# KhaoulaAguech/pl-fem-vectoriel

Hardware: AMD Instinct MI355X
Metric: eigenmodes/sec (assembly+solve), 7-core P2 mesh, 10 modes; |Δn_eff| vs ref (higher is better)
Workload: dtype f64

## Files before the change

### pl_fem_vectoriel_amd/csrc/device.h

```cpp
#pragma once
#include <hip/hip_runtime.h>

#include <cstdint>
#include <functional>
#include <string>
#include <type_traits>
#include <vector>

#include "../../include/plfem.h"
#include "internal.h"
#include "plan.h"

namespace plfem {

constexpr size_t PIN_POST = 0;
constexpr size_t PIN_RESID = 2048;
constexpr size_t PIN_CORE_QP = 4000;
constexpr size_t PIN_COUNTERS = 4096;
constexpr int PIN_COUNTERS_N = 2 * 4;
constexpr size_t PIN_CORES = 6144;
constexpr size_t PIN_PROJ = 8192;
static_assert(PIN_POST + 5 * PLFEM_MAX_NCV <= PIN_RESID, "pinned layout: post-processing sums");
static_assert(PIN_RESID + 3 * PLFEM_MAX_NCV <= PIN_CORE_QP, "pinned layout: residual check");
static_assert(PIN_CORE_QP + 1 <= PIN_COUNTERS, "pinned layout: core-point counter");
// ... 21 lines not shown
  } while (0)

struct plfem_ctx {
  const plfem::Symbolic* S = nullptr;
  const plfem::LaunchPlan* plan = nullptr;
  int device = 0;
  hipStream_t stream = nullptr;
  std::string err;
  int nv = 0, ne = 0, N = 0, nnz = 0, nsolve = 0, L = 0, nfronts = 0, max_ncv = 0;
  int dpn = 2, sh = 1;
  int64_t fnodes_total = 0;
  int64_t n2 = 0;
  int32_t* d_forder = nullptr;
  plfem::FrontRec* d_frec = nullptr;
  int2* d_tiles = nullptr;
  plfem::SweepJob* d_blk = nullptr;
  int32_t *d_tsorted = nullptr, *d_edof = nullptr, *d_rowptr = nullptr, *d_colind = nullptr;
  int32_t *d_slot_row = nullptr, *d_nptr = nullptr, *d_nadj = nullptr, *d_interior = nullptr;
  uint8_t* d_nloc = nullptr;
  uint8_t* d_bmask = nullptr;
  double* d_doflocs = nullptr;
  int32_t *d_fs2 = nullptr, *d_fm = nullptr;
  int64_t *d_fnode_ptr = nullptr, *d_foff = nullptr;
  int32_t *d_fnodes = nullptr, *d_cinv0 = nullptr, *d_cinv1 = nullptr;
  int32_t *d_epos = nullptr, *d_leaf_elem_ptr = nullptr, *d_leaf_elems = nullptr;
  double* d_cores = nullptr;
  double* d_elem = nullptr;
  double* d_vals[PLFEM_BLK_COUNT] = {nullptr};
  double* d_front = nullptr;
  double* d_schur = nullptr;
  int64_t arena_doubles = 0;
  int64_t* d_soff = nullptr;
  double* d_fvec = nullptr;
  double *d_u0 = nullptr, *d_u1 = nullptr;
  double* d_xl = nullptr;
  int32_t* d_npos = nullptr;
  int32_t* d_prow = nullptr;
  double *d_wbuf = nullptr, *d_rbuf = nullptr;
  double* d_dinv = nullptr;
  double* d_delta = nullptr;
  double* d_fvec2 = nullptr;
  int32_t* d_counters = nullptr;
  double *d_V = nullptr, *d_BV = nullptr, *d_V2 = nullptr, *d_BV2 = nullptr;
  double *d_w = nullptr, *d_bw = nullptr, *d_t1 = nullptr, *d_t2 = nullptr;
  double *d_hblk = nullptr, *d_G = nullptr, *d_Rinv = nullptr;
  double *d_h = nullptr, *d_hacc = nullptr, *d_partial = nullptr, *d_scal = nullptr, *d_S = nullptr;
  double* d_Hcols = nullptr;
  uint8_t* d_coremask = nullptr;
  double* d_post = nullptr;
  size_t post_doubles = 0;
  size_t partial_doubles = 0;
  double* h_pinned = nullptr;
  size_t h_pinned_bytes = 0;
  double* h_staging = nullptr;
  size_t h_staging_bytes = 0;
  double* h_slots = nullptr;
  char* slab = nullptr;
  size_t slab_off = 0, slab_bytes = 0;
  bool own_slab = false;
  int64_t workspace_need = 0;
  bool assembled = false, factored = false;
  hipEvent_t ev_step[2] = {nullptr, nullptr};
  bool defer_sync = false;
  hipStream_t copy_stream = nullptr;
  hipEvent_t ev_copy = nullptr;
  hipEvent_t ev_upload = nullptr;
  bool upload_pending = false;
  bool prof_on = false;
  unsigned prof_toggle = 0;
  int prof_n = 0, prof_max = 0;
  std::vector<hipEvent_t> prof_ev;
  std::vector<int> prof_slot;
  std::vector<double> prof_rbytes;
  int refine_steps = 0;
  void (*test_post_factor)(plfem_ctx*) = nullptr;
  double test_perturb = 0.0;
  int max_block_p = plfem::BLOCK_P;
  double sigma = 0.0;
  hipEvent_t ev[plfem::PH_COUNT][2] = {};
  bool ev_used[plfem::PH_COUNT] = {};
  double* modes_dev = nullptr;
  int modes_k = 0;
};

namespace {
template <class Owner>
int check_launch(Owner* owner, const char* what) {
  const hipError_t e = hipGetLastError();
  if (e == hipSuccess) return PLFEM_OK;
  owner->err = std::string(what) + ": " + hipGetErrorString(e);
  return PLFEM_EHIP;
}

int wait_for_upload(plfem_ctx* c) {
  if (!c->upload_pending) return PLFEM_OK;
  HIP_TRY(c, hipStreamWaitEvent(c->stream, c->ev_upload, 0));
  c->upload_pending = false;
  return PLFEM_OK;
}

hipError_t phase_begin(plfem_ctx* c, plfem::Phase ph) { return hipEventRecord(c->ev[ph][0], c->stream); }
hipError_t phase_end(plfem_ctx* c, plfem::Phase ph) {
  const hipError_t e = hipEventRecord(c->ev[ph][1], c->stream);
  if (e == hipSuccess) c->ev_used[ph] = true;
  return e;
}
double phase_us(const plfem_ctx* c, plfem::Phase ph) {
  float ms = 0;
  return (c->ev_used[ph] && hipEventElapsedTime(&ms, c->ev[ph][0], c->ev[ph][1]) == hipSuccess) ? ms * 1e3 : 0.0;
}
}

namespace plfem {

inline int prof_open(plfem_ctx* c, int slot, double bytes) {
  if (!c->prof_on || c->prof_n >= c->prof_max) return -1;
  while ((int)c->prof_ev.size() < 2 * (c->prof_n + 1)) {
    hipEvent_t e;
    if (hipEventCreate(&e) != hipSuccess) return -1;
    c->prof_ev.push_back(e);
  }
  const int id = c->prof_n++;
  c->prof_slot.push_back(slot);
  c->prof_rbytes.push_back(bytes);
  (void)hipEventRecord(c->prof_ev[2 * id], c->stream);
  return id;
}
inline void prof_close(plfem_ctx* c, int id) {
  if (id >= 0) (void)hipEventRecord(c->prof_ev[2 * id + 1], c->stream);
}

template <int V, int... Rest, class F>
inline void with_constant(int v, F&& f) {
  if constexpr (sizeof...(Rest) == 0) f(std::integral_constant<int, V>());
  else if (v == V) f(std::integral_constant<int, V>());
  else with_constant<Rest...>(v, f);
}

inline int ceil_div(int64_t a, int64_t b) { return (int)((a + b - 1) / b); }
inline int basis_cols(int max_ncv) { return max_ncv + 1 + BLOCK_P; }
inline int proj_cols(int max_ncv) { return basis_cols(max_ncv) + 8; }

void launch_element_matrices(plfem_ctx* c, int ncore, double eps_core, double eps_clad, double k0, double alpha_p);
void launch_element_matrices_scalar(plfem_ctx* c, int ncore, double eps_core, double eps_clad, double k0);
double launch_delta_eps_mass(plfem_ctx* c, int ncore, double eps_core, double eps_clad);
void launch_csr_gather(plfem_ctx* c);
void launch_pattern_fill(plfem_ctx* c);
void launch_spmv(plfem_ctx* c, int which, int P, const double* x, double* y, int64_t ld);
int launch_spmv_b_block_il(plfem_ctx* c, const double* x_interleaved, double* y, int64_t ld, double* gram = nullptr);
inline int spmv_workgroups(int N) { return ceil_div(N, SPMV_WG_ROWS); }
inline size_t gram_partial_doubles(int N) { return (size_t)BLOCK_P * BLOCK_P * spmv_workgroups(N); }
void launch_residuals(plfem_ctx* c, int k, const double* lam_host, const double* evecs, double* out_host);
void launch_factor(plfem_ctx* c, double sigma, int stop_level = -1, int stop_step = 0, int stop_stage = 0);
void launch_solve(plfem_ctx* c, int P, const double* rhs, double* x, int64_t ldx, bool rhs_in_front_order = false);
inline int sweep_ldv(int m) { return (m + 2) & ~1; }
inline size_t sweep_dynamic_lds(int P, int m) { return sizeof(double) * P * sweep_ldv(m); }
inline size_t sweep_lds(int P, int m) { return sweep_dynamic_lds(P, m) + sizeof(double) * 8 * P * 64; }
void solve_refined(plfem_ctx* c, int P, const double* b, double* y, int64_t ld, bool b_in_front_order, int steps, double* ta,
                   double* tb, double* dy);
void launch_panel_dot(plfem_ctx* c, int P, const double* Pm, int ncols, const double* W, int64_t ldw, double* h, int ldh,
                      double* hacc = nullptr, int ldacc = 0);
inline int panel_chunks(int64_t n2) { return ceil_div(n2, PANEL_CHUNK); }
inline size_t panel_dot_partial_doubles(int64_t n2, int ncols) { return (size_t)panel_chunks(n2) * ncols * BLOCK_P; }
void launch_panel_axpy(plfem_ctx* c, int P, const double* Pm, int ncols, const double* H, int ldh, double* W, int64_t ldw,
                       double* w_interleaved = nullptr);
void launch_dot(plfem_ctx* c, const double* a, const double* b, double* out);
void launch_scale_store(plfem_ctx* c, const double* w, const double* bw, const double* beta2, double* v, double* bv,
                        double* beta_out);
void launch_axpby(plfem_ctx* c, int64_t n, double a, const double* x, double b, const double* y, double* z);
void launch_rotate(plfem_ctx* c, const double* V, int m, const double* Smat, int ldS, int p, double* out);
void launch_first_pass_block(plfem_ctx* c, const double* BVm, const double* Vm, int ncols, double* W, int64_t ldw, double* Hout, int ldh);
inline int first_pass_segments(int64_t n2) { return ceil_div(n2, FIRST_ROWS); }
inline size_t first_pass_partial_doubles(int64_t n2) { return (size_t)FIRST_COLS * BLOCK_P * first_pass_segments(n2); }
void launch_chol_from_partials(plfem_ctx* c, int nchunks, double* Tblk, int ldT, double* Rinv);
void launch_chol_block(plfem_ctx* c, const double* G, int ldg, double* Tblk, int ldT, double* Rinv);
void launch_block_scale(plfem_ctx* c, const double* W, const double* BW, int64_t ldw, const double* Rinv, double* Vn,
                        double* BVn, int64_t ldv, const double* exp_src = nullptr, int exp_n = 0, double* exp_dst = nullptr,
                        int32_t* cnt_dst = nullptr, double* bv_front = nullptr);
void launch_start_field(plfem_ctx* c, int nvec, double* out);
void launch_post(plfem_ctx* c, int k, double* evecs, int ncore, double* out_host, double* frac_core, double* modes_int);
void post_enqueue(plfem_ctx* c, int k, double* evecs, int ncore, double* modes_int, const std::function<void(int, int)>* group_done);
void post_finish(plfem_ctx* c, int k, double* out_host, double* frac_core);
void resid_enqueue(plfem_ctx* c, int k, const double* lam_host, const double* evecs);
void resid_finish(plfem_ctx* c, int k, double* out_host);
inline int post_blocks(int N) { return ceil_div(N, POST_ROWS); }
inline size_t post_sum_doubles(int N, int modes) { return (size_t)POST_SUMS * modes * (post_blocks(N) + 1); }
inline size_t resid_sum_doubles(int N, int modes) { return (size_t)RESID_SUMS * modes * (post_blocks(N) + 1); }

}
```

### pl_fem_vectoriel_amd/csrc/kernels_front.hip

```cpp
#include <algorithm>

#include <type_traits>

#include "device.h"

namespace plfem {
namespace {

typedef double v4d __attribute__((ext_vector_type(4)));

__device__ __forceinline__ double* schur_of(int f, const int64_t* __restrict__ soff, double* __restrict__ schur, int64_t arena) {
  const int level = 31 - __clz(f + 1);
  return schur + (level & 1) * arena + soff[f];
}

template <int sh>
__global__ __launch_bounds__(256) void k_leaf_assemble(
    int first_front, int ne, double sigma, const int32_t* __restrict__ fs2, const int32_t* __restrict__ fm,
    const int64_t* __restrict__ foff, const int64_t* __restrict__ soff,
    const int64_t* __restrict__ fnode_ptr, const int32_t* __restrict__ fnodes,
    const int32_t* __restrict__ leaf_elem_ptr, const int32_t* __restrict__ leaf_elems,
    const int32_t* __restrict__ epos, const double* __restrict__ elem, double* __restrict__ front,
    double* __restrict__ schur, int64_t arena) {
  const int lf = blockIdx.x;
  const int f = first_front + lf;
  const int m = fm[f], s2 = fs2[f], b2 = m - s2;
  constexpr int dpn = sh + 1;
  double* F = front + foff[f];
  double* S = schur_of(f, soff, schur, arena);
  auto at = [&](int i, int j) -> int64_t { return j < s2 ? (int64_t)j * m + i : (i >= s2 ? -2 - ((int64_t)(j - s2) * b2 + (i - s2)) : -1); };
  const int tid = threadIdx.x;
  const int32_t* fn = fnodes + fnode_ptr[f];
  for (int q = tid; q < (m >> sh); q += 256)
    if (fn[q] < 0) {
      for (int cc = 0; cc < dpn; ++cc) {
        const int d = dpn * q + cc;
        if (d < s2) F[(int64_t)d * m + d] = 1.0;
        else S[(int64_t)(d - s2) * b2 + (d - s2)] = 1.0;
      }
    }
  __syncthreads();
  constexpr int nd = 6 * dpn;
  const int adof = tid / nd, bdof = tid % nd;
  const int a = adof >> sh, ca = adof & sh, b = bdof >> sh, cb = bdof & sh;
  const bool worker = tid < nd * nd;
  const int blk_a = (ca == 0 && cb == 0) ? PLFEM_BLK_AXX : (ca == 0) ? PLFEM_BLK_AXY : (cb == 0) ? PLFEM_BLK_AYX : PLFEM_BLK_AYY;
  const bool diag_blk = ca == cb;
  constexpr int EB = 8;
  for (int q0 = leaf_elem_ptr[lf]; q0 < leaf_elem_ptr[lf + 1]; q0 += EB) {
    const int nb = min(EB, leaf_elem_ptr[lf + 1] - q0);
    int64_t dst[EB];
    double val[EB];
#pragma unroll
    for (int t = 0; t < EB; ++t) {
      dst[t] = -1;
      val[t] = 0.0;
      if (worker && t < nb) {
        const int e = leaf_elems[q0 + t];
        const int pa = epos[(size_t)(q0 + t) * 6 + a], pb = epos[(size_t)(q0 + t) * 6 + b];
        const double* em = elem + (size_t)e * ELEM_STRIDE + a * 6 + b;
        double v = em[blk_a * 36];
        if (diag_blk) v -= sigma * em[PLFEM_BLK_MINV * 36];
        if (pa >= 0 && pb >= 0) { dst[t] = at(dpn * pa + ca, dpn * pb + cb); val[t] = v; }
      }
    }
#pragma unroll
    for (int t = 0; t < EB; ++t) {
      if (t < nb) {
        if (dst[t] >= 0) F[dst[t]] += val[t];
        else if (dst[t] <= -2) S[-2 - dst[t]] += val[t];
        __syncthreads();
      }
    }
  }
}

template <int sh>
__global__ __launch_bounds__(256) void k_front_gather(
    const int2* __restrict__ tiles, const int32_t* __restrict__ fs2, const int32_t* __restrict__ fm,
    const int64_t* __restrict__ foff, const int64_t* __restrict__ soff, const int64_t* __restrict__ fnode_ptr,
    const int32_t* __restrict__ fnodes, const int32_t* __restrict__ cinv0, const int32_t* __restrict__ cinv1,
    double* __restrict__ front, double* __restrict__ schur, int64_t arena) {
  const int2 job = tiles[blockIdx.x];
  const int f = job.x;
  const int m = fm[f], s2 = fs2[f], b2 = m - s2;
  constexpr int dpn = sh + 1;
  const int i = (job.y & 0xffff) * 64 + (threadIdx.x & 63);
  const int j0 = ((job.y >> 16) * 4 + (threadIdx.x >> 6)) * 16;
  if (i >= m || j0 >= m) return;
  if (j0 >= s2 && i < s2) return;
  const int64_t np = fnode_ptr[f];
  const int qi = i >> sh, ci = i & sh;
  const int c0i = cinv0[np + qi], c1i = cinv1[np + qi];
  const bool dummy_i = fnodes[np + qi] < 0;
  const int ch0 = 2 * f + 1, ch1 = 2 * f + 2;
  const int b0 = fm[ch0] - fs2[ch0], b1 = fm[ch1] - fs2[ch1];
  const double* S0 = schur_of(ch0, soff, schur, arena);
  const double* S1 = schur_of(ch1, soff, schur, arena);
  double* F = front + foff[f];
  double* S = schur_of(f, soff, schur, arena);
  int c0j[16 >> sh], c1j[16 >> sh];
#pragma unroll
  for (int q = 0; q < (16 >> sh); ++q) {
    c0j[q] = cinv0[np + (j0 >> sh) + q];
    c1j[q] = cinv1[np + (j0 >> sh) + q];
  }
  double v[16];
#pragma unroll
  for (int jj = 0; jj < 16; ++jj) {
    const int cj = jj & sh, q = jj >> sh;
    double a = 0.0, b = 0.0;
    if (c0i >= 0 && c0j[q] >= 0) {
      const int bi = dpn * c0i + ci, bj = dpn * c0j[q] + cj;
      a = S0[(int64_t)min(bi, bj) * b0 + max(bi, bj)];
    }
    if (c1i >= 0 && c1j[q] >= 0) {
      const int bi = dpn * c1i + ci, bj = dpn * c1j[q] + cj;
      b = S1[(int64_t)min(bi, bj) * b1 + max(bi, bj)];
    }
    v[jj] = a + b;
  }
#pragma unroll
  for (int jj = 0; jj < 16; ++jj) {
    const int j = j0 + jj;
    const double val = (dummy_i && i == j) ? 1.0 : v[jj];
    if (j0 < s2) F[(int64_t)j * m + i] = val;
    else S[(int64_t)(j - s2) * b2 + (i - s2)] = val;
  }
}

__device__ __forceinline__ double fast_rcp(double d) {
  double r = __builtin_amdgcn_rcp(d);
  r = fma(fma(-d, r, 1.0), r, r);
  return fma(fma(-d, r, 1.0), r, r);
}

__device__ __forceinline__ double lane_xor16(double v, bool odd_row) {
  const int lo = __double2loint(v), hi = __double2hiint(v);
  const auto a = __builtin_amdgcn_permlane16_swap(lo, lo, false, false);
  const auto b = __builtin_amdgcn_permlane16_swap(hi, hi, false, false);
  return __hiloint2double(odd_row ? b[0] : b[1], odd_row ? a[0] : a[1]);
}

__device__ __forceinline__ void pair_step(double a, double b, double c, double thr, double rep, bool past_first, bool past_second,
                                          double y0, double y1, const double (&ra)[4], const double (&rb)[4],
                                          double (&v)[4], double& d0, double& d1, double& od, int& nper) {
  const double p = b * b;
  const double det = fma(a, c, -p) - fma(b, b, -p);
  const double s = fmax(fmax(fabs(a), fabs(c)), fabs(b));
  if (p * fabs(det) <= (a * a) * (s * s)) {
    if (__builtin_expect(!(fabs(a) >= thr), 0)) {
      a = (a < 0.0) ? -rep : rep;
      nper += 1;
    }
    const double r1 = fast_rcp(a);
    const double g = b * r1;
    double d2 = fma(-g, b, c);
    if (__builtin_expect(!(fabs(d2) >= thr), 0)) {
      d2 = (d2 < 0.0) ? -rep : rep;
      nper += 1;
    }
    const double r2 = fast_rcp(d2);
    const double l0 = past_first ? y0 * r1 : 0.0;
    const double l1 = past_second ? fma(-l0, b, y1) * r2 : 0.0;
#pragma unroll
    for (int cc = 0; cc < 4; ++cc) v[cc] = fma(-l1, fma(-g, ra[cc], rb[cc]), fma(-l0, ra[cc], v[cc]));
    d0 = r1;
    d1 = r2;
    od = 0.0;
    asm volatile("" ::: "memory");
  } else {
    double dt = det;
    if (__builtin_expect(!(fabs(dt) >= thr * s), 0)) {
      dt = (dt < 0.0) ? -rep * s : rep * s;
      nper += 1;
    }
    const double rd = fast_rcp(dt);
    const double x11 = c * rd, x12 = -b * rd, x22 = a * rd;
    const double l0 = past_second ? fma(y0, x11, y1 * x12) : 0.0;
    const double l1 = past_second ? fma(y0, x12, y1 * x22) : 0.0;
#pragma unroll
    for (int cc = 0; cc < 4; ++cc) v[cc] = fma(-l1, rb[cc], fma(-l0, ra[cc], v[cc]));
    d0 = x11;
    d1 = x22;
    od = x12;
    asm volatile("" ::: "memory");
  }
}

struct PivotLds {
  double row[2][2][NB];
  double col[2][2][NB];
  double rmax[NB];
};

__device__ __forceinline__ void ldl_pivot_block(const double* src, int64_t ld, int nbk, int tid,
                                                double (*tile)[NB + 1], double* __restrict__ sDd, double* __restrict__ sDo,
                                                PivotLds& S, int32_t* __restrict__ counters) {
  static_assert(NB == 32, "thread map of ldl_pivot_block");
  const int i = tid & 31, cg = tid >> 5;
  double v[4];
  double rmax = 0.0;
#pragma unroll
  for (int cc = 0; cc < 4; ++cc) {
    const int c = 4 * cg + cc;
    v[cc] = (i < nbk && c < nbk) ? src[(int64_t)c * ld + i] : (i == c ? 1.0 : 0.0);
    rmax = fmax(rmax, fabs(v[cc]));
  }
  __syncthreads();
  tile[cg][i] = rmax;
  __syncthreads();
  if (tid < NB) {
    double r = 0.0;
#pragma unroll
    for (int g = 0; g < 8; ++g) r = fmax(r, fmax(tile[g][tid], tile[g][tid ^ 1]));
    S.rmax[tid] = r;
  }
  double dd = 1.0, od = 0.0;
  int nper = 0;
#pragma unroll
  for (int q = 0; q < NB / 2; ++q) {
    const int k = 2 * q, cgk = k >> 2, pc = k & 3, buf = q & 1;
    if (k >= nbk) break;
    if (cg == cgk) {
      S.col[buf][0][i] = v[pc];
// ... 366 lines not shown
  {
    PanelOperands po;
    po.load(tile, sDd, sDo, nbn, lr, lk);
    po.rows(bq, nbn, t0, m, ibase0 + lr, lk, Wn, Yn, F);
  }
  for (int ibase = ibase0 + n_pan * 64; ibase < m; ibase += n_pan * 64) {
    int ml = m;
    int64_t pl = pbase;
    asm volatile("" : "+s"(ml), "+s"(pl) : : "memory");
    strip(ibase, bq, std::false_type(), ml, pl);
    asm volatile("" ::: "memory");
    PanelOperands po;
    po.load(tile, sDd, sDo, nbn, lr, lk);
    po.rows(bq, nbn, t0, ml, ibase + lr, lk, wbuf_next + pl, rbuf_next + pl, F);
  }
}

template <int MODE>
__global__ __launch_bounds__(256) __attribute__((amdgpu_waves_per_eu(3, 3))) void k_ldl_update(
    int un, int n_inv, int n_look, int n_pan, const int2* __restrict__ tiles, const int32_t* __restrict__ forder,
    const FrontRec* __restrict__ frec, int kb,
    const int32_t* __restrict__ fs2, const int32_t* __restrict__ fm, const int64_t* __restrict__ foff,
    const int64_t* __restrict__ soff, const int64_t* __restrict__ fnode_ptr, double* __restrict__ front,
    double* __restrict__ schur, int64_t arena, const double* __restrict__ dinv, double* __restrict__ dinv_next,
    double* __restrict__ delta, const double* __restrict__ wbuf, const double* __restrict__ rbuf,
    const double* __restrict__ wbuf_prev, const double* __restrict__ rbuf_prev, double* __restrict__ wbuf_next,
    double* __restrict__ rbuf_next, int32_t* __restrict__ counters) {
  int bid = blockIdx.x;
  if (bid < n_look * n_pan) {
    const FrontRec R = frec[bid / n_pan];
    ldl_column_block<MODE>(R, bid % n_pan, n_pan, kb, front, dinv_next, delta, wbuf, rbuf, wbuf_prev, rbuf_prev, wbuf_next,
                           rbuf_next, counters);
    return;
  }
  bid -= n_look * n_pan;
  if (bid < un) {
    ldl_update_tile<MODE>(tiles[bid], kb, fs2, fm, foff, soff, fnode_ptr, front, schur, arena, wbuf, rbuf, wbuf_prev, rbuf_prev);
    return;
  }
  bid -= un;
  const int f = forder[bid / (n_inv + 1)];
  const int sub = bid % (n_inv + 1);
  if (sub < n_inv) {
    __shared__ double part[3 * 8 * 64];
    ldl_invrow_block(f, sub, kb, fs2, fm, foff, front, dinv, part);
    return;
  }
  const int s2 = fs2[f];
  const int k0 = kb * NB;
  if (k0 >= s2) return;
  const int nbk = min(NB, s2 - k0);
  const int m = fm[f];
  double* F = front + foff[f];
  const double* D = dinv + (int64_t)f * NB * NB;
  for (int q = threadIdx.x; q < NB * NB; q += 256) {
    const int i = q & (NB - 1), c = q >> 5;
    if (i < nbk && c < nbk) F[(int64_t)(k0 + c) * m + (k0 + i)] = (i >= c) ? D[i + c * NB] : D[c + i * NB];
  }
}

__device__ __forceinline__ void mirror_x_block(const int2 job, const int32_t* __restrict__ fs2, const int32_t* __restrict__ fm,
                                               const int64_t* __restrict__ foff, double* __restrict__ front,
                                               double (*tile)[33]) {
  const int f = job.x, k0 = job.y * NB;
  const int m = fm[f], s2 = fs2[f];
  const int nbk = min(NB, s2 - k0);
  double* F = front + foff[f];
  const int tx = threadIdx.x & 31, ty = threadIdx.x >> 5;
  for (int c0 = 0; c0 < k0; c0 += 32) {
    for (int yy = ty; yy < 32; yy += 8)
      tile[yy][tx] = (yy < nbk) ? F[(int64_t)(k0 + yy) * m + c0 + tx] : 0.0;
    __syncthreads();
    for (int yy = ty; yy < 32; yy += 8)
      if (tx < nbk) F[(int64_t)(c0 + yy) * m + k0 + tx] = tile[tx][yy];
    __syncthreads();
  }
}

__global__ __launch_bounds__(256) void k_form_z_mirror(const int2* __restrict__ jobs, int nz, const int32_t* __restrict__ fs2,
                                                       const int32_t* __restrict__ fm, const int64_t* __restrict__ foff,
                                                       double* __restrict__ front) {
  __shared__ double lds[4][32][33];
  const int2 job = jobs[blockIdx.x];
  if ((int)blockIdx.x >= nz) {
    mirror_x_block(job, fs2, fm, foff, front, lds[0]);
    return;
  }
  const int f = job.x;
  const int m = fm[f], s2 = fs2[f];
  const int b2 = m - s2;
  const int wave = threadIdx.x >> 6, lane = threadIdx.x & 63;
  const int b0 = (job.y * 2 + (wave & 1)) * 32;
  const bool rows_on = b0 < b2;
  double* F = front + foff[f];
  double* FZ = F + (int64_t)m * s2;
  const int lr = lane & 15, lk = lane >> 4;
  const bool bv1 = b0 + 16 < b2;
  double (*tile)[33] = lds[wave];
  for (int cstep = 0; cstep < s2; cstep += 64) {
    const int c0 = cstep + 32 * (wave >> 1);
    const bool on = rows_on && c0 < s2;
    const bool cv1 = c0 + 16 < s2;
    v4d acc[2][2];
    for (int tb = 0; tb < 2; ++tb)
      for (int tc = 0; tc < 2; ++tc) acc[tb][tc] = (v4d){0.0, 0.0, 0.0, 0.0};
    if (on) {
      const int cA = c0 + lr, cB = c0 + 16 + lr;
      for (int j0 = c0; j0 < s2; j0 += 16) {
        double a0[4], a1[4], x0[4], x1[4];
#pragma unroll
        for (int t = 0; t < 4; ++t) {
          const int j = j0 + 4 * t + lk;
          a0[t] = F[(int64_t)j * m + s2 + b0 + lr];
          a1[t] = bv1 ? F[(int64_t)j * m + s2 + b0 + 16 + lr] : 0.0;
          x0[t] = (j >= cA) ? F[(int64_t)j * m + cA] : 0.0;
          x1[t] = (cv1 && j >= cB) ? F[(int64_t)j * m + cB] : 0.0;
        }
#pragma unroll
        for (int t = 0; t < 4; ++t) {
          acc[0][0] = __builtin_amdgcn_mfma_f64_16x16x4f64(a0[t], x0[t], acc[0][0], 0, 0, 0);
          acc[0][1] = __builtin_amdgcn_mfma_f64_16x16x4f64(a0[t], x1[t], acc[0][1], 0, 0, 0);
          acc[1][0] = __builtin_amdgcn_mfma_f64_16x16x4f64(a1[t], x0[t], acc[1][0], 0, 0, 0);
          acc[1][1] = __builtin_amdgcn_mfma_f64_16x16x4f64(a1[t], x1[t], acc[1][1], 0, 0, 0);
        }
      }
      for (int tb = 0; tb < 2; ++tb)
        for (int tc = 0; tc < 2; ++tc)
#pragma unroll
          for (int r = 0; r < 4; ++r) {
            const int bb = 16 * tb + lk + 4 * r, cc = 16 * tc + lr;
            tile[cc][bb] = acc[tb][tc][r];
            if ((tb == 0 || bv1) && (tc == 0 || cv1)) FZ[(int64_t)(b0 + bb) * s2 + (c0 + cc)] = acc[tb][tc][r];
          }
    }
    __syncthreads();
    if (on) {
      const int bb = lane & 31;
#pragma unroll 4
      for (int cc = lane >> 5; cc < 32; cc += 2)
        if (b0 + bb < b2 && c0 + cc < s2) F[(int64_t)(c0 + cc) * m + s2 + b0 + bb] = tile[cc][bb];
    }
  }
}

}

void launch_factor(plfem_ctx* c, double sigma, int stop_level, int stop_step, int stop_stage) {
  hipStream_t st = c->stream;
  const LaunchPlan& plan = *c->plan;
  (void)hipMemsetAsync(c->d_counters, 0, 4 * sizeof(int32_t), st);
  for (int lev = c->L; lev >= 0; --lev) {
    const LevelInfo& li = plan.levels[lev];
    if (lev == c->L) {
      const int64_t lo = c->S->foff[li.first], hi = c->S->foff[li.first + li.count];
      (void)hipMemsetAsync(c->d_front + lo, 0, sizeof(double) * (size_t)(hi - lo), st);
      int64_t sch = 0;
      for (int f = li.first; f < li.first + li.count; ++f) {
        const int64_t b2 = (int64_t)c->dpn * c->S->fb[f];
        sch = std::max(sch, c->S->soff[f] + b2 * b2);
      }
      (void)hipMemsetAsync(c->d_schur + (size_t)(lev & 1) * c->arena_doubles, 0, sizeof(double) * (size_t)sch, st);
      with_constant<0, 1>(c->sh, [&](auto sh) {
        hipLaunchKernelGGL(k_leaf_assemble<decltype(sh)::value>, dim3(li.count), dim3(256), 0, st, li.first, c->ne, sigma, c->d_fs2,
                           c->d_fm, c->d_foff, c->d_soff, c->d_fnode_ptr, c->d_fnodes, c->d_leaf_elem_ptr, c->d_leaf_elems, c->d_epos,
                           c->d_elem, c->d_front, c->d_schur, c->arena_doubles);
      });
    } else if (li.gather_n > 0) {
      with_constant<0, 1>(c->sh, [&](auto sh) {
        hipLaunchKernelGGL(k_front_gather<decltype(sh)::value>, dim3(li.gather_n), dim3(256), 0, st, c->d_tiles + li.gather_off,
                           c->d_fs2, c->d_fm, c->d_foff, c->d_soff, c->d_fnode_ptr, c->d_fnodes, c->d_cinv0, c->d_cinv1, c->d_front,
                           c->d_schur, c->arena_doubles);
      });
    }
    if (lev == stop_level && stop_stage == 0) return;
    const int steps = (li.max_s2 + NB - 1) / NB;
    const int32_t* ford = c->d_forder + li.first;
    const FrontRec* frec = c->d_frec + li.first;
    const int* hs2 = plan.forder_s2.data() + li.first;
    const int* hpm = plan.forder_maxm.data() + li.first;
    for (int kb = 0; kb < steps; ++kb) {
      const bool stop_here = (lev == stop_level && kb == stop_step);
      const int k0 = kb * NB;
      int nact = 0;
      {
        int lo = 0, hi = li.count;
        while (lo < hi) { int mid = (lo + hi) / 2; if (hs2[mid] > k0) lo = mid + 1; else hi = mid; }
        nact = lo;
      }
      if (nact == 0) break;
      const size_t third = (size_t)2 * plan.level_nodes_max * NB;
      const int64_t base = 2 * c->S->fnode_ptr[li.first] * NB;
      double* wb0 = c->d_wbuf - base;
      double* rb0 = c->d_rbuf - base;
      double* wb = wb0 + (kb % 3) * third;
      double* rb = rb0 + (kb % 3) * third;
      double* wb_prev = wb0 + ((kb + 2) % 3) * third;
      double* rb_prev = rb0 + ((kb + 2) % 3) * third;
      double* wb_next = wb0 + ((kb + 1) % 3) * third;
      double* rb_next = rb0 + ((kb + 1) % 3) * third;
      double* dinv_cur = c->d_dinv + (size_t)(kb & 1) * c->nfronts * NB * NB;
      double* dinv_nxt = c->d_dinv + (size_t)((kb + 1) & 1) * c->nfronts * NB * NB;
      auto panel_wgs = [&](int rows_below, int cap) {
        int n = std::max(1, rows_below > 0 ? (rows_below + 63) / 64 : 0);
        return li.count > 64 ? std::min(n, cap) : n;
      };
      if (kb == 0) {
        const int n_pan0 = panel_wgs(hpm[nact - 1] - 16, 2);
        hipLaunchKernelGGL(k_ldl_first_panel, dim3(nact, n_pan0), dim3(256), 0, st, frec, c->d_front, dinv_cur, c->d_delta, wb, rb,
                           c->d_counters);
      }
      if (stop_here && stop_stage >= 1 && stop_stage <= 2) return;
      const int un = plan.upd_n[li.step0 + kb];
      const int n_inv = kb > 0 ? (k0 + 15) / 16 : 0;
      const int2* ut = c->d_tiles + plan.upd_off[li.step0 + kb];
      int n_look = 0;
      {
        int lo = 0, hi = nact;
        while (lo < hi) { int mid = (lo + hi) / 2; if (hs2[mid] > k0 + NB) lo = mid + 1; else hi = mid; }
        n_look = lo;
      }
      const int cap = li.count >= 1024 ? 1 : 4;
      const int n_pan = n_look > 0 ? panel_wgs(hpm[n_look - 1] - (k0 + NB) - 16, cap) : 1;
      const unsigned gridB = (unsigned)(n_look * n_pan + un + nact * (n_inv + 1));
      with_constant<0, 1>(kb & 1, [&](auto mode) {
        hipLaunchKernelGGL(k_ldl_update<decltype(mode)::value>, dim3(gridB), dim3(256), 0, st, un, n_inv, n_look, n_pan, ut, ford,
                           frec, kb, c->d_fs2, c->d_fm, c->d_foff, c->d_soff, c->d_fnode_ptr, c->d_front, c->d_schur, c->arena_doubles,
                           dinv_cur, dinv_nxt, c->d_delta, wb, rb, mode ? wb_prev : wb, mode ? rb_prev : rb, wb_next, rb_next,
                           c->d_counters);
      });
      if (stop_here && (stop_stage == 3 || stop_stage == 4)) return;
    }
    if (stop_level >= 0 && li.formz_n + li.mirrorx_n > 0)
      hipLaunchKernelGGL(k_form_z_mirror, dim3(li.formz_n + li.mirrorx_n), dim3(256), 0, st, c->d_tiles + li.formz_off, li.formz_n,
                         c->d_fs2, c->d_fm, c->d_foff, c->d_front);
    if (lev == stop_level && stop_stage == 5) return;
  }
  if (stop_level < 0 && plan.formz_all_n + plan.mirrorx_all_n > 0)
    hipLaunchKernelGGL(k_form_z_mirror, dim3(plan.formz_all_n + plan.mirrorx_all_n), dim3(256), 0, st, c->d_tiles + plan.formz_all_off,
                       plan.formz_all_n, c->d_fs2, c->d_fm, c->d_foff, c->d_front);
}

}
```

### pl_fem_vectoriel_amd/csrc/plan.h

```cpp
#pragma once
#include <cstdint>
#include <functional>
#include <memory>
#include <utility>
#include <vector>

namespace plfem {

template <class T>
struct default_init_allocator : std::allocator<T> {
  template <class U>
  struct rebind { using other = default_init_allocator<U>; };
  using std::allocator<T>::allocator;
  template <class U>
  void construct(U* ptr) noexcept { ::new (static_cast<void*>(ptr)) U; }
  template <class U, class... Args>
  void construct(U* ptr, Args&&... args) { ::new (static_cast<void*>(ptr)) U(std::forward<Args>(args)...); }
};

constexpr int NB = 32;
constexpr int PANEL_CHUNK = 1024;
constexpr int FIRST_ROWS = 1024;
constexpr int FIRST_COLS = 8;
constexpr int SPMV_WG_ROWS = 32;
constexpr int POST_ROWS = 256;
constexpr int POST_SUMS = 5;
constexpr int RESID_SUMS = 2;
constexpr int ROW_FORM_MAX_FRONTS = 32;
constexpr int MIX_BIG_S2 = 192;
constexpr int SWEEP_ROW_JOB_FLAG = 1 << 30;
struct alignas(16) SweepJob {
  int32_t f, rb;
  int32_t m, s2;
  int64_t np, npp;
  int64_t foff;
  int64_t reserved;
};
static_assert(sizeof(SweepJob) == 48, "SweepJob layout");
struct alignas(16) FrontRec {
  int32_t f, m, s2, reserved;
  int64_t foff, np;
};
static_assert(sizeof(FrontRec) == 32, "FrontRec layout");
inline int fwd_block_rows(int count) { return count <= 8 ? 8 : count <= ROW_FORM_MAX_FRONTS ? 16 : 64; }
inline int bwd_block_rows(int count, bool leaf) { return leaf ? 64 : count <= ROW_FORM_MAX_FRONTS ? 8 : 16; }
constexpr int BLOCK_P = 4;
constexpr int MAX_CORES = 64;
constexpr int ELEM_FORMS = 8;
constexpr int ELEM_STRIDE = ELEM_FORMS * 36;

struct LevelInfo {
  int first = 0;
  int count = 0;
  int max_m = 0;
  int max_s2 = 0;
  int max_b2 = 0;
  int64_t gather_off = 0, formz_off = 0, mirrorx_off = 0;
  int gather_n = 0, formz_n = 0, mirrorx_n = 0, step0 = 0;
  int fwd_rows = 0, bwd_rows = 0;
  bool fwd_mixed = false;
  int64_t fwd_off = 0, bwd_off = 0;
  int fwd_n = 0, bwd_n = 0;
  double sweep_bytes = 0;
  double sweep_vec_doubles = 0;
};

struct Tile { int32_t x, y; };
static_assert(sizeof(Tile) == 8, "Tile layout");

struct Symbolic;
struct LaunchPlan {
  bool built = false;
  std::vector<int32_t> fs2, fm;
  std::vector<int32_t> forder;
  std::vector<int32_t> forder_s2, forder_maxm;
  std::vector<FrontRec, default_init_allocator<FrontRec>> frec;
  std::vector<LevelInfo> levels;
  std::vector<SweepJob, default_init_allocator<SweepJob>> jobs;
  std::vector<Tile, default_init_allocator<Tile>> tiles;
  std::vector<int64_t> upd_off;
  std::vector<int32_t> upd_n;
  int64_t formz_all_off = 0, mirrorx_all_off = 0;
  int32_t formz_all_n = 0, mirrorx_all_n = 0;
  int64_t level_nodes_max = 0;
  int32_t worst_m = 0;
};
using PlanTasks = std::function<void(int ntasks, const std::function<void(int)>& f)>;
void build_launch_plan(const Symbolic& S, LaunchPlan& P, const PlanTasks& par = {});

}
```

Measured before the change: 527.7.

## Assemble leaf fronts in LDS via hash table and write dense columns directly

Measured after the change: 505.8. 0.959x the previous value.

```diff
diff --git a/pl_fem_vectoriel_amd/csrc/device.h b/pl_fem_vectoriel_amd/csrc/device.h
--- a/pl_fem_vectoriel_amd/csrc/device.h
+++ b/pl_fem_vectoriel_amd/csrc/device.h
@@ -197,6 +197,11 @@
 inline size_t gram_partial_doubles(int N) { return (size_t)BLOCK_P * BLOCK_P * spmv_workgroups(N); }
 void launch_residuals(plfem_ctx* c, int k, const double* lam_host, const double* evecs, double* out_host);
 void launch_factor(plfem_ctx* c, double sigma, int stop_level = -1, int stop_step = 0, int stop_stage = 0);
+inline constexpr size_t leaf_assemble_lds(int dpn) {
+  return sizeof(double) * 36 * LEAF_CHUNK * dpn * dpn + sizeof(uint32_t) * (LEAF_CELLS + LEAF_BITMAP_WORDS) +
+         sizeof(int32_t) * 7 * LEAF_CHUNK + sizeof(uint16_t) * 36 * LEAF_CHUNK + LEAF_PANEL_MAX;
+}
+static_assert(2 * leaf_assemble_lds(2) <= 160 * 1024, "leaf assembly: two workgroups per CU on gfx950");
 void launch_solve(plfem_ctx* c, int P, const double* rhs, double* x, int64_t ldx, bool rhs_in_front_order = false);
 inline int sweep_ldv(int m) { return (m + 2) & ~1; }
 inline size_t sweep_dynamic_lds(int P, int m) { return sizeof(double) * P * sweep_ldv(m); }
diff --git a/pl_fem_vectoriel_amd/csrc/kernels_front.hip b/pl_fem_vectoriel_amd/csrc/kernels_front.hip
--- a/pl_fem_vectoriel_amd/csrc/kernels_front.hip
+++ b/pl_fem_vectoriel_amd/csrc/kernels_front.hip
@@ -14,63 +14,201 @@
   return schur + (level & 1) * arena + soff[f];
 }
 
+__device__ __forceinline__ unsigned leaf_pair_hash(unsigned key) { return (key * 2654435761u) >> (32 - __builtin_ctz(LEAF_CELLS)); }
+
 template <int sh>
-__global__ __launch_bounds__(256) void k_leaf_assemble(
-    int first_front, int ne, double sigma, const int32_t* __restrict__ fs2, const int32_t* __restrict__ fm,
-    const int64_t* __restrict__ foff, const int64_t* __restrict__ soff,
+__global__ __launch_bounds__(LEAF_THREADS) void k_leaf_assemble(
+    int first_front, double sigma, const int32_t* __restrict__ forder, const int32_t* __restrict__ fs2,
+    const int32_t* __restrict__ fm, const int64_t* __restrict__ foff, const int64_t* __restrict__ soff,
     const int64_t* __restrict__ fnode_ptr, const int32_t* __restrict__ fnodes,
     const int32_t* __restrict__ leaf_elem_ptr, const int32_t* __restrict__ leaf_elems,
     const int32_t* __restrict__ epos, const double* __restrict__ elem, double* __restrict__ front,
     double* __restrict__ schur, int64_t arena) {
-  const int lf = blockIdx.x;
-  const int f = first_front + lf;
-  const int m = fm[f], s2 = fs2[f], b2 = m - s2;
   constexpr int dpn = sh + 1;
+  constexpr int dd = dpn * dpn;
+  constexpr unsigned EMPTY = 0xffffffffu;
+  constexpr unsigned short NONE = 0xffff;
+  __shared__ __attribute__((aligned(16))) double vals[36 * LEAF_CHUNK * dd];
+  __shared__ unsigned cells[LEAF_CELLS];
+  __shared__ unsigned bitmap[LEAF_BITMAP_WORDS];
+  __shared__ int32_t spos[6 * LEAF_CHUNK], sel[LEAF_CHUNK];
+  __shared__ unsigned short cslot[36 * LEAF_CHUNK];
+  __shared__ unsigned char spad[LEAF_PANEL_MAX];
+  const int f = forder[blockIdx.x];
+  const int lf = f - first_front;
+  const int m = fm[f], s2 = fs2[f], b2 = m - s2, nn = m >> sh;
   double* F = front + foff[f];
   double* S = schur_of(f, soff, schur, arena);
-  auto at = [&](int i, int j) -> int64_t { return j < s2 ? (int64_t)j * m + i : (i >= s2 ? -2 - ((int64_t)(j - s2) * b2 + (i - s2)) : -1); };
+  const int32_t* fn = fnodes + fnode_ptr[f];
   const int tid = threadIdx.x;
-  const int32_t* fn = fnodes + fnode_ptr[f];
-  for (int q = tid; q < (m >> sh); q += 256)
-    if (fn[q] < 0) {
-      for (int cc = 0; cc < dpn; ++cc) {
-        const int d = dpn * q + cc;
-        if (d < s2) F[(int64_t)d * m + d] = 1.0;
-        else S[(int64_t)(d - s2) * b2 + (d - s2)] = 1.0;
-      }
-    }
-  __syncthreads();
+  auto s_first_row = [](int jj) { return max(0, (jj & ~15) - 16); };
+  auto entry = [&](int i, int j) -> double* {
+    if (j < s2) return F + (int64_t)j * m + i;
+    const int ii = i - s2, jj = j - s2;
+    return ii >= s_first_row(jj) ? S + (int64_t)jj * b2 + ii : nullptr;
+  };
+  auto pair_of = [&](unsigned c, int& pa, int& pb) {
+    const unsigned t = c / 36, ab = c - 36 * t, a = ab / 6;
+    pa = spos[6 * t + a];
+    pb = spos[6 * t + (ab - 6 * a)];
+  };
+  auto find = [&](int pa, int pb) -> unsigned {
+    unsigned h = leaf_pair_hash((unsigned)pb * nn + pa);
+    for (;;) {
+      const unsigned c = cells[h];
+      int qa, qb;
+      pair_of(c, qa, qb);
+      if (qa == pa && qb == pb) return c;
+      h = (h + 1) & (LEAF_CELLS - 1);
+    }
+  };
   constexpr int nd = 6 * dpn;
-  const int adof = tid / nd, bdof = tid % nd;
+  const int grp = tid / 160, gl = tid - 160 * grp;
+  const int adof = gl / nd, bdof = gl % nd;
   const int a = adof >> sh, ca = adof & sh, b = bdof >> sh, cb = bdof & sh;
-  const bool worker = tid < nd * nd;
+  const bool worker = grp < 3 && gl < nd * nd;
   const int blk_a = (ca == 0 && cb == 0) ? PLFEM_BLK_AXX : (ca == 0) ? PLFEM_BLK_AXY : (cb == 0) ? PLFEM_BLK_AYX : PLFEM_BLK_AYY;
   const bool diag_blk = ca == cb;
-  constexpr int EB = 8;
-  for (int q0 = leaf_elem_ptr[lf]; q0 < leaf_elem_ptr[lf + 1]; q0 += EB) {
-    const int nb = min(EB, leaf_elem_ptr[lf + 1] - q0);
-    int64_t dst[EB];
-    double val[EB];
-#pragma unroll
-    for (int t = 0; t < EB; ++t) {
-      dst[t] = -1;
-      val[t] = 0.0;
-      if (worker && t < nb) {
-        const int e = leaf_elems[q0 + t];
-        const int pa = epos[(size_t)(q0 + t) * 6 + a], pb = epos[(size_t)(q0 + t) * 6 + b];
-        const double* em = elem + (size_t)e * ELEM_STRIDE + a * 6 + b;
-        double v = em[blk_a * 36];
-        if (diag_blk) v -= sigma * em[PLFEM_BLK_MINV * 36];
-        if (pa >= 0 && pb >= 0) { dst[t] = at(dpn * pa + ca, dpn * pb + cb); val[t] = v; }
-      }
-    }
-#pragma unroll
-    for (int t = 0; t < EB; ++t) {
-      if (t < nb) {
-        if (dst[t] >= 0) F[dst[t]] += val[t];
-        else if (dst[t] <= -2) S[-2 - dst[t]] += val[t];
+  const int qbeg = leaf_elem_ptr[lf], qend = leaf_elem_ptr[lf + 1];
+  for (int q0 = qbeg; q0 == qbeg || q0 < qend; q0 += LEAF_CHUNK) {
+    const bool first_pass = q0 == qbeg;
+    const int nq = max(0, min(LEAF_CHUNK, qend - q0));
+    for (int h = tid; h < LEAF_CELLS; h += LEAF_THREADS) cells[h] = EMPTY;
+    for (int x = tid; x < 6 * nq; x += LEAF_THREADS) spos[x] = epos[(size_t)q0 * 6 + x];
+    if (tid < nq) sel[tid] = leaf_elems[q0 + tid];
+    __syncthreads();
+    for (int c = tid; c < 36 * nq; c += LEAF_THREADS) {
+      int pa, pb;
+      pair_of(c, pa, pb);
+      unsigned slot = NONE;
+      if (pa >= 0 && pb >= 0) {
+        unsigned h = leaf_pair_hash((unsigned)pb * nn + pa);
+        for (;;) {
+          const unsigned old = atomicCAS(&cells[h], EMPTY, (unsigned)c);
+          if (old == EMPTY) { slot = c; break; }
+          int qa, qb;
+          pair_of(old, qa, qb);
+          if (qa == pa && qb == pb) { slot = old; break; }
+          h = (h + 1) & (LEAF_CELLS - 1);
+        }
+      }
+      cslot[c] = (unsigned short)slot;
+    }
+    __syncthreads();
+    for (int c = tid; c < 36 * nq; c += LEAF_THREADS) {
+      if (cslot[c] == c) {
+        int pa, pb;
+        pair_of(c, pa, pb);
+#pragma unroll
+        for (int x = 0; x < dd; ++x) {
+          double v0 = 0.0;
+          if (!first_pass) {
+            const double* p = entry(dpn * pa + (x & sh), dpn * pb + (x >> sh));
+            if (p) v0 = __hip_atomic_load(p, __ATOMIC_RELAXED, __HIP_MEMORY_SCOPE_AGENT);
+          }
+          vals[c * dd + x] = v0;
+        }
+      }
+    }
+    __syncthreads();
+    constexpr int EG = (LEAF_CHUNK + 2) / 3;
+    {
+      int dst[EG];
+      double val[EG];
+#pragma unroll
+      for (int u = 0; u < EG; ++u) {
+        const int t = 3 * u + grp;
+        dst[u] = -1;
+        val[u] = 0.0;
+        if (worker && t < nq) {
+          const unsigned slot = cslot[36 * t + 6 * a + b];
+          const double* em = elem + (size_t)sel[t] * ELEM_STRIDE + a * 6 + b;
+          double v = em[blk_a * 36];
+          if (diag_blk) v -= sigma * em[PLFEM_BLK_MINV * 36];
+          if (slot != NONE) { dst[u] = slot * dd + cb * dpn + ca; val[u] = v; }
+        }
+      }
+#pragma unroll
+      for (int u = 0; u < EG; ++u) {
+#pragma unroll
+        for (int g = 0; g < 3; ++g) {
+          if (3 * u + g < nq) {
+            if (grp == g && dst[u] >= 0) vals[dst[u]] += val[u];
+            __syncthreads();
+          }
+        }
+      }
+    }
+    if (!first_pass) {
+      for (int c = tid; c < 36 * nq; c += LEAF_THREADS) {
+        if (cslot[c] == c) {
+          int pa, pb;
+          pair_of(c, pa, pb);
+#pragma unroll
+          for (int x = 0; x < dd; ++x) {
+            double* p = entry(dpn * pa + (x & sh), dpn * pb + (x >> sh));
+            if (p) *p = vals[c * dd + x];
+          }
+        }
+      }
+    } else {
+      const int wave = tid >> 6, lane = tid & 63;
+      const int hm = m >> 1;
+      constexpr int npr = 2 / dpn;
+      const int wc = max(1, min(nn, 32 * LEAF_BITMAP_WORDS / nn));
+      for (int c0 = 0; c0 < nn; c0 += wc) {
+        const int c1 = min(nn, c0 + wc);
+        for (int w = tid; w < ((c1 - c0) * nn + 31) / 32; w += LEAF_THREADS) bitmap[w] = 0;
+        if (tid < c1 - c0) spad[tid] = fn[c0 + tid] < 0;
         __syncthreads();
-      }
+        for (int h = tid; h < LEAF_CELLS; h += LEAF_THREADS) {
+          const unsigned c = cells[h];
+          if (c == EMPTY) continue;
+          int pa, pb;
+          pair_of(c, pa, pb);
+          if (pb < c0 || pb >= c1) continue;
+          const int bit = (pb - c0) * nn + pa;
+          atomicOr(&bitmap[bit >> 5], 1u << (bit & 31));
+        }
+        __syncthreads();
+        for (int pj = c0 + wave; pj < c1; pj += LEAF_THREADS / 64) {
+          const int j0 = dpn * pj;
+          const bool in_f = j0 < s2;
+          const int r0 = in_f ? 0 : (s2 + s_first_row(j0 - s2)) >> 1;
+          double* col = in_f ? F + (int64_t)j0 * m : S + (int64_t)(j0 - s2) * b2 - s2;
+          const int ld = in_f ? m : b2;
+          const bool pad_j = spad[pj - c0];
+          for (int r = r0 + lane; r < hm; r += 64) {
+            double o[dpn][2];
+#pragma unroll
+            for (int x = 0; x < dpn; ++x) o[x][0] = o[x][1] = 0.0;
+#pragma unroll
+            for (int k = 0; k < npr; ++k) {
+              const int pi = npr * r + k;
+              const int bit = (pj - c0) * nn + pi;
+              if ((bitmap[bit >> 5] >> (bit & 31)) & 1) {
+                const unsigned c = find(pi, pj);
+#pragma unroll
+                for (int xb = 0; xb < dpn; ++xb)
+#pragma unroll
+                  for (int xa = 0; xa < dpn; ++xa) o[xb][k * dpn + xa] = vals[c * dd + xb * dpn + xa];
+              }
+              if (pad_j && pi == pj) {
+#pragma unroll
+                for (int xa = 0; xa < dpn; ++xa) o[xa][k * dpn + xa] = 1.0;
+              }
+            }
+#pragma unroll
+            for (int xb = 0; xb < dpn; ++xb)
+              *reinterpret_cast<double2*>(col + (int64_t)xb * ld + 2 * r) = make_double2(o[xb][0], o[xb][1]);
+          }
+        }
+        __syncthreads();
+      }
+    }
+    if (q0 + LEAF_CHUNK < qend) {
+      __threadfence();
+      __syncthreads();
     }
   }
 }
@@ -743,18 +881,10 @@
   for (int lev = c->L; lev >= 0; --lev) {
     const LevelInfo& li = plan.levels[lev];
     if (lev == c->L) {
-      const int64_t lo = c->S->foff[li.first], hi = c->S->foff[li.first + li.count];
-      (void)hipMemsetAsync(c->d_front + lo, 0, sizeof(double) * (size_t)(hi - lo), st);
-      int64_t sch = 0;
-      for (int f = li.first; f < li.first + li.count; ++f) {
-        const int64_t b2 = (int64_t)c->dpn * c->S->fb[f];
-        sch = std::max(sch, c->S->soff[f] + b2 * b2);
-      }
-      (void)hipMemsetAsync(c->d_schur + (size_t)(lev & 1) * c->arena_doubles, 0, sizeof(double) * (size_t)sch, st);
       with_constant<0, 1>(c->sh, [&](auto sh) {
-        hipLaunchKernelGGL(k_leaf_assemble<decltype(sh)::value>, dim3(li.count), dim3(256), 0, st, li.first, c->ne, sigma, c->d_fs2,
-                           c->d_fm, c->d_foff, c->d_soff, c->d_fnode_ptr, c->d_fnodes, c->d_leaf_elem_ptr, c->d_leaf_elems, c->d_epos,
-                           c->d_elem, c->d_front, c->d_schur, c->arena_doubles);
+        hipLaunchKernelGGL(k_leaf_assemble<decltype(sh)::value>, dim3(li.count), dim3(LEAF_THREADS), 0, st, li.first, sigma,
+                           c->d_forder + li.first, c->d_fs2, c->d_fm, c->d_foff, c->d_soff, c->d_fnode_ptr, c->d_fnodes,
+                           c->d_leaf_elem_ptr, c->d_leaf_elems, c->d_epos, c->d_elem, c->d_front, c->d_schur, c->arena_doubles);
       });
     } else if (li.gather_n > 0) {
       with_constant<0, 1>(c->sh, [&](auto sh) {
diff --git a/pl_fem_vectoriel_amd/csrc/plan.h b/pl_fem_vectoriel_amd/csrc/plan.h
--- a/pl_fem_vectoriel_amd/csrc/plan.h
+++ b/pl_fem_vectoriel_amd/csrc/plan.h
@@ -46,6 +46,14 @@
 inline int bwd_block_rows(int count, bool leaf) { return leaf ? 64 : count <= ROW_FORM_MAX_FRONTS ? 8 : 16; }
 constexpr int BLOCK_P = 4;
 constexpr int MAX_CORES = 64;
+constexpr int LEAF_CHUNK = 50;
+constexpr int LEAF_CELLS = 4096;
+constexpr int LEAF_BITMAP_WORDS = 512;
+constexpr int LEAF_PANEL_MAX = 128;
+constexpr int LEAF_THREADS = 512;
+static_assert((LEAF_CELLS & (LEAF_CELLS - 1)) == 0 && LEAF_CELLS >= 2 * 36 * LEAF_CHUNK, "leaf assembly: hash table load");
+static_assert(LEAF_PANEL_MAX * LEAF_PANEL_MAX >= 32 * LEAF_BITMAP_WORDS && LEAF_PANEL_MAX <= LEAF_THREADS, "leaf assembly: bitmap panel");
+static_assert(36 * LEAF_CHUNK < 0xffff && LEAF_THREADS >= 3 * 160, "leaf assembly: 16-bit slot numbers, three lane groups");
 constexpr int ELEM_FORMS = 8;
 constexpr int ELEM_STRIDE = ELEM_FORMS * 36;
 
```
